# wlsdzyzl/OnePiece

Hardware: AMD Instinct MI355X
Metric: RGB-D frames/sec fused (640x480, 5 mm voxel TSDF) (higher is better)
Workload: dtype f32

## Files before the change

### onepiece_amd/csrc/integrate.hip

```cpp
#include "volume_core.hpp"

namespace {

typedef unsigned int kc_v2u __attribute__((ext_vector_type(2)));

__device__ __forceinline__ void voxel_load(const float* p, float& s, float& w, float& c0, float& c1, float& c2) {
    s = p[0]; w = p[kVox]; c0 = p[2 * kVox]; c1 = p[3 * kVox]; c2 = p[4 * kVox];
}
__device__ __forceinline__ void voxel_store(float* p, float s, float w, float c0, float c1, float c2) {
    p[0] = s; p[kVox] = w; p[2 * kVox] = c0; p[3 * kVox] = c1; p[4 * kVox] = c2;
}
template <bool PLAIN, bool LEAN = false>
__device__ __forceinline__ void voxel_update(float& s, float& w, float& c0, float& c1, float& c2, float new_sdf, unsigned rgba, const float* s_c255) {
    const float n0 = s_c255[rgba & 0xffu], n1 = s_c255[(rgba >> 8) & 0xffu], n2 = s_c255[(rgba >> 16) & 0xffu];
    if (PLAIN) {
        const float wv = LEAN ? w : ((s >= 1 || w <= 0) ? 0.0f : w);
        const float ps = wv * s, p0 = wv * c0, p1 = wv * c1, p2 = wv * c2;
        const float wsum = wv + 1.0f;
        const float y = __builtin_amdgcn_rcpf(wsum);
        const float ns = ps + 1.0f * new_sdf;
        const float m0 = p0 + 1.0f * n0, m1 = p1 + 1.0f * n1, m2 = p2 + 1.0f * n2;
        float qs = div_int_rcp(ns, wsum, y), q0 = div_int_rcp(m0, wsum, y), q1 = div_int_rcp(m1, wsum, y), q2 = div_int_rcp(m2, wsum, y);
        const bool slow = LEAN ? !(fabsf(ns) >= 0x1p-60f) : ((wsum > 0x1p19f) | !(fabsf(ns) >= 0x1p-60f));
        if (__builtin_expect(__builtin_amdgcn_ballot_w64(slow) != 0ull, 0)) {
            if (slow) { qs = ns / wsum; q0 = m0 / wsum; q1 = m1 / wsum; q2 = m2 / wsum; }
        }
        s = qs; c0 = q0; c1 = q1; c2 = q2;
        w = wsum;
    } else if (!(s >= 1 || w <= 0)) {
        const float wsum = w + 1.0f;
        s = (w * s + 1.0f * new_sdf) / wsum;
        c0 = (w * c0 + 1.0f * n0) / wsum;
        c1 = (w * c1 + 1.0f * n1) / wsum;
        c2 = (w * c2 + 1.0f * n2) / wsum;
        w = wsum;
    } else {
        s = new_sdf; w = 1.0f; c0 = n0; c1 = n1; c2 = n2;
    }
}

__device__ __forceinline__ void voxel_revert(bool hit, float& s, float& w, float& c0, float& c1, float& c2, float new_sdf, unsigned rgba, const float* s_c255, bool& can,
                                             bool& zero) {
    can = hit & !(s >= 1 || w <= 0) & (w >= 1);
    const float rw = w + (-1.0f);
    zero = rw == 0;
    if (!can) return;
    const float n0 = s_c255[rgba & 0xffu], n1 = s_c255[(rgba >> 8) & 0xffu], n2 = s_c255[(rgba >> 16) & 0xffu];
    if (zero) {
        s = 999.0f; w = 0.0f; c0 = -1.0f; c1 = -1.0f; c2 = -1.0f;
    } else {
        s = (w * s + (-1.0f) * new_sdf) / rw;
        c0 = (w * c0 + (-1.0f) * n0) / rw;
        c1 = (w * c1 + (-1.0f) * n1) / rw;
        c2 = (w * c2 + (-1.0f) * n2) / rw;
        w = rw;
    }
}

#ifdef KC_TRACE
__device__ unsigned long long g_kc_trace[4096 * 4 * 8];
#define KC_T(K) do { const unsigned long long now_ = __builtin_amdgcn_s_memtime(); kt_[K] += now_ - kt_last_; kt_last_ = now_; } while (0)
#define KC_N(K, V) do { kt_[K] += (V); } while (0)
#else
#define KC_T(K) do { } while (0)
#define KC_N(K, V) do { } while (0)
#endif
template <bool FAST, bool PLAIN, int ZT, bool SUMF = false, bool LEAN = false, bool G2D = false, bool SIGNED = false>
__global__ __launch_bounds__(512 / ZT, (SUMF ? KC_SUM_MIN_WAVES : SIGNED ? KC_SIGNED_MIN_WAVES : KC_COL_MIN_WAVES)) void k_integrate(BatchInv B, CamParams C, VolView V, const uint2* __restrict__ pimg, State* st,
                                                                            int n_frames, unsigned long long* __restrict__ upd_partial,
                                                                            unsigned long long* __restrict__ sel_partial, unsigned long long* __restrict__ chg_partial,
                                                                            unsigned plain_from, unsigned* __restrict__ rc_sum, unsigned rc_stamp, bmask_t sign,
                                                                            unsigned long long* __restrict__ dei_partial) {
    static_assert(!SIGNED || !(PLAIN || SUMF || LEAN), "the PLAIN and LEAN hypotheses do not survive a weight of -1");
    constexpr int kWaves = 8 / ZT;
    constexpr bool kSummaries = !SUMF && !SIGNED;
    constexpr bool kWCount = LEAN && !SUMF;
    __shared__ unsigned s_cnt[kWaves][SIGNED ? 5 : 2];
    __shared__ unsigned s_sign[2][kWaves];
    __shared__ float s_c255[256];
    __shared__ unsigned s_next[2];
    const unsigned long long t_in = __builtin_amdgcn_s_memtime();
#ifdef KC_TRACE
    unsigned long long kt_[8] = {0, 0, 0, 0, 0, 0, 0, 0}, kt_last_ = t_in;
#endif
    for (unsigned k = blockIdx.x * blockDim.x + threadIdx.x; k < (unsigned)(kMaxBatch * kAccSlots * 8); k += gridDim.x * blockDim.x) (&st->acc[0][0][0])[k] = 0u;
    if (st->overflow & 3u) return;
    const int tid = threadIdx.x, lane = tid & 63, zg = tid >> 6;
    if (!SUMF) for (int k = tid; k < 256; k += blockDim.x) s_c255[k] = (float)k / 255.0f;
    const unsigned npix = (unsigned)(C.width * C.height);
    const float half = C.res / 2;
    const float ox = (float)(lane & 7) * C.res + half;
    const float oy = (float)(lane >> 3) * C.res + half;
    const float __attribute__((address_space(4)))* kargs =
        (const float __attribute__((address_space(4)))*)__builtin_amdgcn_kernarg_segment_ptr();
    (void)B;
    unsigned upd = 0, sel = 0, chg = 0, nblk = 0;
    unsigned neg_hit = 0, neg_can = 0, rst = 0;
    const bool eighths = n_frames >= KC_STEAL_MIN_FRAMES;
    constexpr unsigned kChunkLog2 = 5u, kChunk = 1u << kChunkLog2;
    const unsigned n0 = st->n_blist < V.max_blocks ? st->n_blist : V.max_blocks;
    const unsigned n_chunks = (n0 + kChunk - 1u) >> kChunkLog2;
    const unsigned per0 = eighths ? (n0 + (unsigned)kKcShares - 1u) / (unsigned)kKcShares : ((n_chunks + (unsigned)kKcShares - 1u) / (unsigned)kKcShares) << kChunkLog2;
    unsigned xcd = blockIdx.x % (unsigned)kKcShares;
    for (;;) {
    unsigned* ctr = &st->kc_next[xcd * 16u];
    if (tid == 0) s_next[0] = atomicAdd(ctr, 1u);
    __syncthreads();
    unsigned slot = 0u;
    for (unsigned j = s_next[0]; j < per0;) {
        if (tid == 0) s_next[slot ^ 1u] = atomicAdd(ctr, 1u);
        const unsigned b = eighths ? xcd * per0 + j : (((j >> kChunkLog2) * (unsigned)kKcShares + xcd) << kChunkLog2) + (j & (kChunk - 1u));
        KC_T(0);
        const int tslot = b < n0 ? V.blist[b] : -1;
        const int idx = tslot >= 0 ? V.tvals[tslot] : -1;
        KC_N(6, 1);
        if (idx >= 0) {
            const bmask_t mask = V.bmask[tslot];
            if (zg == 0) { sel += mask_popc(mask); ++nblk; }
            const int kx = V.keys[3 * idx], ky = V.keys[3 * idx + 1], kz = V.keys[3 * idx + 2];
            float* vox = V.pool + (size_t)idx * kBlockFloats + (zg * ZT) * 64 + lane;
            float s[ZT], w[ZT], c0[ZT], c1[ZT], c2[ZT], pz[ZT];
#pragma unroll
            for (int z = 0; z < ZT; ++z) {
                if (!SUMF) voxel_load(vox + z * 64, s[z], w[z], c0[z], c1[z], c2[z]);
                pz[z] = ((float)kz * 8.0f) * C.res + ((float)(zg * ZT + z) * C.res + half);
            }
            const float px = ((float)kx * 8.0f) * C.res + ox;
            const float py = ((float)ky * 8.0f) * C.res + oy;
            float w0[ZT];
#pragma unroll
            for (int z = 0; z < ZT; ++z) w0[z] = kWCount ? w[z] : 0.0f;
            unsigned changed = 0u;
            unsigned long long changed_m[ZT];
#pragma unroll
            for (int z = 0; z < ZT; ++z) changed_m[z] = 0ull;
            float ssum[ZT];
            unsigned acc02[ZT], acc1n[ZT];
#pragma unroll
            for (int z = 0; z < ZT; ++z) { ssum[z] = 0.0f; acc02[z] = 0u; acc1n[z] = 0u; }
            auto project = [&](int f, kc_v2u (&rec)[ZT], float (&zc)[ZT]) {
                int fo = f;
                asm volatile("" : "+s"(fo));
                const float __attribute__((address_space(4)))* M = kargs + fo * 12;
                const char* fbase = (const char*)pimg + (unsigned)fo * (npix * 8u);
                const __amdgpu_buffer_rsrc_t frame = __builtin_amdgcn_make_buffer_rsrc((void*)fbase, 0, (int)(npix * 8u), 0x00020000);
                const px_v4i frame2d = gather2d_rsrc(fbase, C.width, C.height);
                const float a0 = M[0] * px + M[1] * py, a1 = M[4] * px + M[5] * py, a2 = M[8] * px + M[9] * py;
#pragma unroll
                for (int z = 0; z < ZT; ++z) {
                    const float q0 = (a0 + M[2] * pz[z]) + M[3] * 1.0f;
                    const float q1 = (a1 + M[6] * pz[z]) + M[7] * 1.0f;
                    const float q2 = (a2 + M[10] * pz[z]) + M[11] * 1.0f;
                    zc[z] = q2;
                    if (G2D) {
                        int u, v;
                        project_pixel_uv<FAST>(C, q0, q1, q2, u, v);
                        rec[z] = gather2d(frame2d, u, v, C.width);
                    } else {
                        const int pix = project_pixel<FAST>(C, q0, q1, q2);
                        rec[z] = __builtin_amdgcn_raw_buffer_load_b64(frame, pix * 8, 0, 0);
                    }
                }
            };
            const bool plain_block = PLAIN || (unsigned)idx >= plain_from;
            auto apply = [&](const kc_v2u (&rec)[ZT], const float (&zc)[ZT], auto plain_c, bool negative) {
                constexpr bool kPlain = decltype(plain_c)::value;
#pragma unroll
                for (int z = 0; z < ZT; ++z) {
                    const float d = __uint_as_float(rec[z].x);
                    const float new_sdf = d - zc[z];
                    const bool seen = d > 0, near = fabsf(new_sdf) < C.trunc, hit = seen & near;
                    if constexpr (SIGNED) {
                        if (negative) {
                            bool can, zero;
                            voxel_revert(hit, s[z], w[z], c0[z], c1[z], c2[z], new_sdf, rec[z].y, s_c255, can, zero);
                            const unsigned long long m_can = __builtin_amdgcn_ballot_w64(can);
                            neg_hit += (unsigned)__builtin_popcountll(__builtin_amdgcn_ballot_w64(seen) & __builtin_amdgcn_ballot_w64(near));
                            neg_can += (unsigned)__builtin_popcountll(m_can);
                            rst += (unsigned)__builtin_popcountll(m_can & __builtin_amdgcn_ballot_w64(zero));
                            changed_m[z] |= m_can;
                            continue;
                        }
                    }
                    if (kWCount) {
                        if (hit) voxel_update<true, true>(s[z], w[z], c0[z], c1[z], c2[z], new_sdf, rec[z].y, s_c255);
                        continue;
                    }
                    const unsigned long long hits = __builtin_amdgcn_ballot_w64(seen) & __builtin_amdgcn_ballot_w64(near);
                    upd += (unsigned)__builtin_popcountll(hits);
                    if (SUMF) {
                        ssum[z] += hit ? new_sdf : 0.0f;
                        const unsigned t = hit ? rec[z].y : 0u;
                        acc02[z] += t & 0x00ff00ffu;
                        acc1n[z] += (t >> 8) & 0x00ff00ffu;
                    } else {
                        changed_m[z] |= hits;
                        if (hit) voxel_update<kPlain, kPlain && LEAN>(s[z], w[z], c0[z], c1[z], c2[z], new_sdf, rec[z].y, s_c255);
                    }
                }
            };
            kc_v2u recA[ZT], recB[ZT];
            float zcA[ZT], zcB[ZT];
            bool negA = false, negB = false;
#ifdef KC_TRACE
            { float keep_ = px + py + pz[0]; if (!SUMF) keep_ += s[0]; asm volatile("" :: "v"(keep_)); KC_T(1); }
#endif
            auto frames = [&](auto plain_c) {
                bmask_t m = mask;
                if (!m) return;
                int f = mask_ctz(m); m &= m - 1u;
                project(f, recA, zcA);
                if constexpr (SIGNED) negA = ((sign >> f) & 1u) != 0u;
                for (;;) {
                    const bool more1 = m != 0u;
                    if (more1) {
                        f = mask_ctz(m); m &= m - 1u; project(f, recB, zcB);
                        if constexpr (SIGNED) negB = ((sign >> f) & 1u) != 0u;
                    }
                    apply(recA, zcA, plain_c, negA);
                    if (!more1) break;
                    const bool more2 = m != 0u;
                    if (more2) {
                        f = mask_ctz(m); m &= m - 1u; project(f, recA, zcA);
                        if constexpr (SIGNED) negA = ((sign >> f) & 1u) != 0u;
                    }
                    apply(recB, zcB, plain_c, negB);
                    if (!more2) break;
                }
            };
            if constexpr (SIGNED) frames(std::false_type{});
            else if (SUMF || PLAIN || plain_block) frames(std::true_type{}); else frames(std::false_type{});
            KC_T(2); KC_N(7, mask_popc(mask));
            if (SUMF) {
#pragma unroll
                for (int z = 0; z < ZT; ++z)
                    if (acc1n[z] >> 16) voxel_load(vox + z * 64, s[z], w[z], c0[z], c1[z], c2[z]);
#pragma unroll
                for (int z = 0; z < ZT; ++z) {
                    const unsigned cnt = acc1n[z] >> 16;
                    if (cnt) {
                        changed |= 1u << z;
                        const bool valid = !(s[z] >= 1 || w[z] <= 0);
                        const float wv = valid ? w[z] : 0.0f, nf = (float)cnt, wsum = wv + nf;
                        const float b0 = (float)(acc02[z] & 0xffffu) / 255.0f, b1 = (float)(acc1n[z] & 0xffffu) / 255.0f, b2 = (float)(acc02[z] >> 16) / 255.0f;
                        s[z] = ((valid ? wv * s[z] : 0.0f) + ssum[z]) / wsum;
                        c0[z] = ((valid ? wv * c0[z] : 0.0f) + b0) / wsum;
                        c1[z] = ((valid ? wv * c1[z] : 0.0f) + b1) / wsum;
                        c2[z] = ((valid ? wv * c2[z] : 0.0f) + b2) / wsum;
                        w[z] = wsum;
                    }
                }
            }
            if (kWCount) {
#pragma unroll
                for (int z = 0; z < ZT; ++z) {
                    const bool wrote = w[z] != w0[z];
                    upd += (unsigned)(w[z] - w0[z]);
                    chg += (unsigned)__builtin_popcountll(__builtin_amdgcn_ballot_w64(wrote));
                    if (wrote) voxel_store(vox + z * 64, s[z], w[z], c0[z], c1[z], c2[z]);
                }
            } else {
#pragma unroll
                for (int z = 0; z < ZT; ++z)
                    if (SUMF ? ((changed >> z) & 1u) != 0u : ((changed_m[z] >> lane) & 1ull) != 0ull) voxel_store(vox + z * 64, s[z], w[z], c0[z], c1[z], c2[z]);
                if (SUMF) chg += (unsigned)__popc(changed);
                else {
#pragma unroll
                    for (int z = 0; z < ZT; ++z) chg += (unsigned)__builtin_popcountll(changed_m[z]);
                }
            }
            if (kSummaries && rc_sum) {
                bool neg = false, pos = false;
#pragma unroll
                for (int z = 0; z < ZT; ++z) { const bool obs = w[z] > 0; neg |= obs && s[z] <= 0; pos |= obs && s[z] > 0; }
                const unsigned f = (__builtin_amdgcn_ballot_w64(neg) ? 1u : 0u) | (__builtin_amdgcn_ballot_w64(pos) ? 2u : 0u);
                if (lane == 0) s_sign[slot][zg] = f;
            }
        }
        KC_T(3);
        __syncthreads();
        KC_T(4);
        if (tslot >= 0 && tid == 0) V.bmask[tslot] = (bmask_t)0;
        if (kSummaries && rc_sum && idx >= 0 && tid == 0) {
            unsigned f = 0u;
#pragma unroll
            for (int k = 0; k < kWaves; ++k) f |= s_sign[slot][k];
            rc_sum[idx] = (rc_stamp << 2) | f;
        }
        slot ^= 1u;
        j = s_next[slot];
    }
    if (!eighths) break;
    __syncthreads();
    if (tid < 64) {
        unsigned left = 0u;
        if (tid < kKcShares) {
            const unsigned c = __hip_atomic_load(&st->kc_next[(unsigned)tid * 16u], __ATOMIC_RELAXED, __HIP_MEMORY_SCOPE_AGENT);
            left = c < per0 ? per0 - c : 0u;
        }
        unsigned key = ((left < 0x7fffffu ? left : 0x7fffffu) << 8) | (unsigned)tid;
#pragma unroll
        for (int o = 32; o > 0; o >>= 1) { const unsigned x = __shfl_xor(key, o, 64); key = x > key ? x : key; }
        if (tid == 0) s_next[0] = key;
    }
    __syncthreads();
    const unsigned key = s_next[0];
    if ((key >> 8) == 0u) break;
    xcd = key & 0xffu;
    __syncthreads();
    }
#ifdef KC_TRACE
    KC_T(5);
    if (lane == 0 && blockIdx.x < 4096) for (int k = 0; k < 8; ++k) g_kc_trace[((size_t)blockIdx.x * 4 + zg) * 8 + k] = kt_[k];
#endif
    if (SUMF) chg = wave_sum(chg);
    if (kWCount) upd = wave_sum(upd);
    if (lane == 0) { s_cnt[zg][0] = upd; s_cnt[zg][1] = chg; }
    if constexpr (SIGNED) if (lane == 0) { s_cnt[zg][2] = neg_can - rst; s_cnt[zg][3] = rst; s_cnt[zg][4] = neg_hit - neg_can; }
    __syncthreads();
    if (tid == 0) {
        unsigned t = 0, c = 0;
        for (int k = 0; k < kWaves; ++k) { t += s_cnt[k][0]; c += s_cnt[k][1]; }
        const unsigned slot_c = blockIdx.x % (unsigned)kPartialGrid;
        if constexpr (SIGNED) {
            unsigned d[3] = {0, 0, 0};
            for (int k = 0; k < kWaves; ++k)
                for (int q = 0; q < 3; ++q) d[q] += s_cnt[k][2 + q];
            atomicAdd(&dei_partial[kDeiReverted + slot_c], (unsigned long long)d[0]);
            atomicAdd(&dei_partial[kDeiReset + slot_c], (unsigned long long)d[1]);
            atomicAdd(&dei_partial[kDeiSkipped + slot_c], (unsigned long long)d[2]);
            if (blockIdx.x == 0) dei_partial[kDeiFrames] += (unsigned long long)mask_popc(sign);
        }
        atomicAdd(&upd_partial[slot_c], (unsigned long long)t);
        atomicAdd(&sel_partial[slot_c], (unsigned long long)sel);
        atomicAdd(&chg_partial[slot_c], (unsigned long long)c);
        atomicAdd(&chg_partial[kPartialGrid + slot_c], (unsigned long long)nblk);
        if (blockIdx.x == 0) { st->stat_frames += (unsigned long long)n_frames; st->stat_launches += 1ull; }
        atomicMax(&st->kc_t[blockIdx.x % (unsigned)kKcTSlots], (unsigned long long)__builtin_amdgcn_s_memtime() - t_in);
    }
}

__global__ __launch_bounds__(256) void k_debug_voxel_update(const float* __restrict__ s, const float* __restrict__ w, const float* __restrict__ c0, const float* __restrict__ c1,
                                                            const float* __restrict__ c2, const float* __restrict__ new_sdf, const unsigned* __restrict__ rgba, long long n,
                                                            float* __restrict__ out_fast, float* __restrict__ out_ref) {
    __shared__ float s_c255[256];
    s_c255[threadIdx.x] = (float)threadIdx.x / 255.0f;
    __syncthreads();
    const long long i = blockIdx.x * 256ll + threadIdx.x;
    if (i >= n) return;
    float a[5] = {s[i], w[i], c0[i], c1[i], c2[i]}, b[5] = {a[0], a[1], a[2], a[3], a[4]};
    voxel_update<true>(a[0], a[1], a[2], a[3], a[4], new_sdf[i], rgba[i], s_c255);
    voxel_update<false>(b[0], b[1], b[2], b[3], b[4], new_sdf[i], rgba[i], s_c255);
    for (int k = 0; k < 5; ++k) { out_fast[5 * i + k] = a[k]; out_ref[5 * i + k] = b[k]; }
}
__global__ void k_debug_rcp(const float* __restrict__ x, long long n, float* __restrict__ out) {
    const long long i = blockIdx.x * 256ll + threadIdx.x;
    if (i < n) out[i] = __builtin_amdgcn_rcpf(x[i]);
}
__global__ void k_debug_gather2d(const uint2* __restrict__ img, int width, int height, int frame, int column_test, const int* __restrict__ uv, long long n,
                                 uint2* __restrict__ out) {
    const long long i = blockIdx.x * 256ll + threadIdx.x;
    if (i >= n) return;
    int fo = frame;
    asm volatile("" : "+s"(fo));
    const px_v4i rsrc = gather2d_rsrc(img + (size_t)fo * ((size_t)width * height), width, height);
    const px_v2u r = column_test ? gather2d(rsrc, uv[2 * i], uv[2 * i + 1], width) : op_struct_buffer_load_b64(rsrc, uv[2 * i + 1], uv[2 * i] << 3, 0, 0);
    out[i] = make_uint2(r.x, r.y);
}

}

namespace opv {

bool vol_fusion_keeps_summaries(const op_volume* v) {
    const bool sum_form = v->update_mode == OP_VOLUME_UPDATE_SUM_FORM && v->trunc < 1.0f;
    return !sum_form && v->rc_sum != nullptr && v->rc_cap >= v->max_blocks && (v->content_gen >> 30) == v->rc_sum_epoch;
}

enum { kUpdSum, kUpdLean, kUpdPlain, kUpdGeneral, kUpdSigned };
enum { kGatExact, kGatFastRaw, kGatFast2d };
template <int UPD, int GAT>
void launch_kc(op_volume* v, const BatchInv& I, const CamParams& C, int nf, bmask_t sign, unsigned* rc_sum) {
    constexpr bool kSum = UPD == kUpdSum, kSigned = UPD == kUpdSigned;
    constexpr int kZt = kSum ? KC_ZT_SUM : KC_ZT;
    hipLaunchKernelGGL((k_integrate<GAT != kGatExact, (UPD <= kUpdPlain), kZt, kSum, UPD == kUpdLean, GAT == kGatFast2d, kSigned>),
                       dim3(kSum ? kColGridSum : kSigned ? kSignedGrid : kColGrid), dim3(512 / kZt), 0, v->stream, I, C, v->view(), (const uint2*)v->pimg, v->state, nf,
                       v->upd_partial, v->sel_partial, v->chg_partial, v->plain_from, rc_sum, (unsigned)(v->content_gen & 0x3fffffffull), sign, v->dei_partial);
}

void launch_integrate(op_volume* v, const BatchInv& I, const CamParams& C, int nf, bmask_t sign) {
    const bool sum_form = !sign && v->update_mode == OP_VOLUME_UPDATE_SUM_FORM && v->trunc < 1.0f;
    unsigned* rc_sum = !sign && vol_fusion_keeps_summaries(v) ? v->rc_sum : nullptr;
    if (sum_form || !(v->trunc <= 0.5f)) v->lean_ok = false;
    v->lean_frames += (uint64_t)nf;
    const bool lean = v->plain && v->lean_ok && v->lean_frames <= (1ull << 19);
    const int upd = sign ? kUpdSigned : sum_form ? kUpdSum : lean ? kUpdLean : v->plain ? kUpdPlain : kUpdGeneral;
    const int gat = !C.fast_px ? kGatExact : gather2d_fits(C.width) ? kGatFast2d : kGatFastRaw;
    typedef void (*launch_fn)(op_volume*, const BatchInv&, const CamParams&, int, bmask_t, unsigned*);
    static const launch_fn table[5][3] = {
        {launch_kc<kUpdSum, kGatExact>, launch_kc<kUpdSum, kGatFastRaw>, launch_kc<kUpdSum, kGatFast2d>},
        {launch_kc<kUpdLean, kGatExact>, launch_kc<kUpdLean, kGatFastRaw>, launch_kc<kUpdLean, kGatFast2d>},
        {launch_kc<kUpdPlain, kGatExact>, launch_kc<kUpdPlain, kGatFastRaw>, launch_kc<kUpdPlain, kGatFast2d>},
        {launch_kc<kUpdGeneral, kGatExact>, launch_kc<kUpdGeneral, kGatFastRaw>, launch_kc<kUpdGeneral, kGatFast2d>},
        {launch_kc<kUpdSigned, kGatExact>, launch_kc<kUpdSigned, kGatFastRaw>, launch_kc<kUpdSigned, kGatFast2d>}};
    table[upd][gat](v, I, C, nf, sign, rc_sum);
}

void kc_trace_dump(op_volume* v) {
#ifdef KC_TRACE
    if (hipSetDevice(v->device) == hipSuccess && hipDeviceSynchronize() == hipSuccess) {
        const int nw = kColGrid * (8 / KC_ZT);
        std::vector<unsigned long long> t((size_t)4096 * 4 * 8);
        if (hipMemcpyFromSymbol(t.data(), HIP_SYMBOL(g_kc_trace), t.size() * 8) == hipSuccess) {
            double sum[8] = {0}, mx[8] = {0};
            for (int w = 0; w < nw; ++w)
                for (int k = 0; k < 8; ++k) { const double d = (double)t[(size_t)w * 8 + k]; sum[k] += d; mx[k] = std::max(mx[k], d); }
            const double n = nw;
            fprintf(stderr, "kc trace (shader cycles per wave of the last launch, %d waves; mean/max): draw+list %.0f/%.0f metadata+voxels %.0f/%.0f frames %.0f/%.0f stores %.0f/%.0f barrier %.0f/%.0f tail %.0f/%.0f | blocks %.1f/%.0f frames applied %.0f/%.0f\n",
                    nw, sum[0] / n, mx[0], sum[1] / n, mx[1], sum[2] / n, mx[2], sum[3] / n, mx[3], sum[4] / n, mx[4], sum[5] / n, mx[5], sum[6] / n, mx[6], sum[7] / n, mx[7]);
        }
    }
#else
    (void)v;
#endif
#ifdef OP_PX_TRACE
    unsigned long long pw[2] = {0, 0};
    if (hipSetDevice(v->device) == hipSuccess && hipDeviceSynchronize() == hipSuccess && hipMemcpyFromSymbol(pw, HIP_SYMBOL(g_px_waves), sizeof(pw)) == hipSuccess)
        fprintf(stderr, "px trace (k_integrate, since load): %llu wave-projections, %llu took the exact fallback (%.3f %%)\n", pw[0], pw[1],
                pw[0] ? 100.0 * (double)pw[1] / (double)pw[0] : 0.0);
#endif
}

}

extern "C" {

int op_debug_voxel_update(const float* s, const float* w, const float* c0, const float* c1, const float* c2, const float* new_sdf, const unsigned* rgba, long long n,
                          float* out_fast, float* out_ref) {
    if (!s || !w || !c0 || !c1 || !c2 || !new_sdf || !rgba || !out_fast || !out_ref) return fail(OP_ERR_INVALID, "null argument");
    if (n < 0 || n > (1ll << 28)) return fail(OP_ERR_INVALID, "n out of range [0, 2^28]");
    OP_TRY(op::use_device(0));
    if (n == 0) return OP_OK;
    const size_t N = (size_t)n;
    float* d_in = nullptr;
    float* d_out = nullptr;
    OP_HIP(op::cached_malloc((void**)&d_in, 7 * N * 4));
    hipError_t e = op::cached_malloc((void**)&d_out, 10 * N * 4);
    const void* src[7] = {s, w, c0, c1, c2, new_sdf, rgba};
    for (int k = 0; k < 7 && e == hipSuccess; ++k) e = hipMemcpy(d_in + k * N, src[k], N * 4, hipMemcpyHostToDevice);
    if (e == hipSuccess) {
        hipLaunchKernelGGL(k_debug_voxel_update, dim3((unsigned)((N + 255) / 256)), dim3(256), 0, 0, (const float*)d_in, (const float*)(d_in + N), (const float*)(d_in + 2 * N),
                           (const float*)(d_in + 3 * N), (const float*)(d_in + 4 * N), (const float*)(d_in + 5 * N), (const unsigned*)(d_in + 6 * N), n, d_out, d_out + 5 * N);
        e = hipMemcpy(out_fast, d_out, 5 * N * 4, hipMemcpyDeviceToHost);
        if (e == hipSuccess) e = hipMemcpy(out_ref, d_out + 5 * N, 5 * N * 4, hipMemcpyDeviceToHost);
    }
    op::cached_free(d_in);
    if (d_out) op::cached_free(d_out);
    if (e != hipSuccess) return fail(OP_ERR_HIP, "op_debug_voxel_update failed: %s", hipGetErrorString(e));
    return OP_OK;
}

int op_debug_rcp(const float* x, long long n, float* out) {
    if (!x || !out) return fail(OP_ERR_INVALID, "null argument");
    if (n < 0 || n > (1ll << 28)) return fail(OP_ERR_INVALID, "n out of range [0, 2^28]");
    OP_TRY(op::use_device(0));
    if (n == 0) return OP_OK;
    const size_t N = (size_t)n;
    float* d = nullptr;
    OP_HIP(op::cached_malloc((void**)&d, 2 * N * 4));
    hipError_t e = hipMemcpy(d, x, N * 4, hipMemcpyHostToDevice);
    if (e == hipSuccess) {
        hipLaunchKernelGGL(k_debug_rcp, dim3((unsigned)((N + 255) / 256)), dim3(256), 0, 0, (const float*)d, n, d + N);
        e = hipMemcpy(out, d + N, N * 4, hipMemcpyDeviceToHost);
    }
    op::cached_free(d);
    if (e != hipSuccess) return fail(OP_ERR_HIP, "op_debug_rcp failed: %s", hipGetErrorString(e));
    return OP_OK;
}

double op_debug_px_rcp_err(void) { return kPxRcpErr; }

int op_debug_gather2d(const unsigned* images, int width, int height, int n_frames, int frame, int column_test, const int* uv, long long n, unsigned* out) {
    if (!images || !uv || !out) return fail(OP_ERR_INVALID, "null argument");
    if (width <= 0 || !gather2d_fits(width) || height <= 0 || n_frames <= 0 || frame < 0 || frame >= n_frames || (long long)width * height * n_frames > (1ll << 24))
        return fail(OP_ERR_INVALID, "op_debug_gather2d: rows of 1 .. %d pixels, a frame of the stack, at most 2^24 pixels in all", kGather2dMaxWidth);
    if (n < 0 || n > (1ll << 24)) return fail(OP_ERR_INVALID, "n out of range [0, 2^24]");
    for (long long i = 0; i < 2 * n; ++i)
        if (uv[i] < -(1 << 23) || uv[i] >= (1 << 23)) return fail(OP_ERR_INVALID, "op_debug_gather2d: coordinates in [-2^23, 2^23)");
    if (!column_test)
        for (long long i = 0; i < n; ++i) {
            const long long rec = ((long long)frame * height + uv[2 * i + 1]) * width + uv[2 * i];
            if (rec < 0 || rec >= (long long)width * height * n_frames) return fail(OP_ERR_INVALID, "op_debug_gather2d: without the column test every address must lie in the stack");
        }
    OP_TRY(op::use_device(0));
    if (n == 0) return OP_OK;
    const size_t N = (size_t)n, img_bytes = (size_t)width * height * n_frames * 8;
    char* d = nullptr;
    OP_HIP(op::cached_malloc((void**)&d, img_bytes + 16 * N));
    hipError_t e = hipMemcpy(d, images, img_bytes, hipMemcpyHostToDevice);
    if (e == hipSuccess) e = hipMemcpy(d + img_bytes, uv, 8 * N, hipMemcpyHostToDevice);
    if (e == hipSuccess) {
        hipLaunchKernelGGL(k_debug_gather2d, dim3((unsigned)((N + 255) / 256)), dim3(256), 0, 0, (const uint2*)d, width, height, frame, column_test, (const int*)(d + img_bytes), n,
                           (uint2*)(d + img_bytes + 8 * N));
        e = hipMemcpy(out, d + img_bytes + 8 * N, 8 * N, hipMemcpyDeviceToHost);
    }
    op::cached_free(d);
    if (e != hipSuccess) return fail(OP_ERR_HIP, "op_debug_gather2d failed: %s", hipGetErrorString(e));
    return OP_OK;
}

}
```

Before: 58200.

## Map each wave onto an 8x4x2 voxel sub-box instead of one z-slice

```diff
diff --git a/onepiece_amd/csrc/integrate.hip b/onepiece_amd/csrc/integrate.hip
--- a/onepiece_amd/csrc/integrate.hip
+++ b/onepiece_amd/csrc/integrate.hip
@@ -1,4 +1,5 @@
 #include "volume_core.hpp"
+#include "kc_lanes.hpp"
 
 namespace {
 
@@ -89,8 +90,9 @@
     if (!SUMF) for (int k = tid; k < 256; k += blockDim.x) s_c255[k] = (float)k / 255.0f;
     const unsigned npix = (unsigned)(C.width * C.height);
     const float half = C.res / 2;
-    const float ox = (float)(lane & 7) * C.res + half;
-    const float oy = (float)(lane >> 3) * C.res + half;
+    const int lx = kc_lanes::vx<ZT>(zg, 0, lane), ly = kc_lanes::vy<ZT>(zg, 0, lane), lz = kc_lanes::vz<ZT>(zg, 0, lane);
+    const float ox = (float)lx * C.res + half;
+    const float oy = (float)ly * C.res + half;
     const float __attribute__((address_space(4)))* kargs =
         (const float __attribute__((address_space(4)))*)__builtin_amdgcn_kernarg_segment_ptr();
     (void)B;
@@ -118,12 +120,12 @@
             const bmask_t mask = V.bmask[tslot];
             if (zg == 0) { sel += mask_popc(mask); ++nblk; }
             const int kx = V.keys[3 * idx], ky = V.keys[3 * idx + 1], kz = V.keys[3 * idx + 2];
-            float* vox = V.pool + (size_t)idx * kBlockFloats + (zg * ZT) * 64 + lane;
+            float* vox = V.pool + (size_t)idx * kBlockFloats + (lx + 8 * ly + 64 * lz);
             float s[ZT], w[ZT], c0[ZT], c1[ZT], c2[ZT], pz[ZT];
 #pragma unroll
             for (int z = 0; z < ZT; ++z) {
-                if (!SUMF) voxel_load(vox + z * 64, s[z], w[z], c0[z], c1[z], c2[z]);
-                pz[z] = ((float)kz * 8.0f) * C.res + ((float)(zg * ZT + z) * C.res + half);
+                if (!SUMF) voxel_load(vox + z * kc_lanes::kSlotStride, s[z], w[z], c0[z], c1[z], c2[z]);
+                pz[z] = ((float)kz * 8.0f) * C.res + ((float)(lz + z * kc_lanes::kBZ) * C.res + half);
             }
             const float px = ((float)kx * 8.0f) * C.res + ox;
             const float py = ((float)ky * 8.0f) * C.res + oy;
@@ -234,7 +236,7 @@
             if (SUMF) {
 #pragma unroll
                 for (int z = 0; z < ZT; ++z)
-                    if (acc1n[z] >> 16) voxel_load(vox + z * 64, s[z], w[z], c0[z], c1[z], c2[z]);
+                    if (acc1n[z] >> 16) voxel_load(vox + z * kc_lanes::kSlotStride, s[z], w[z], c0[z], c1[z], c2[z]);
 #pragma unroll
                 for (int z = 0; z < ZT; ++z) {
                     const unsigned cnt = acc1n[z] >> 16;
@@ -257,12 +259,12 @@
                     const bool wrote = w[z] != w0[z];
                     upd += (unsigned)(w[z] - w0[z]);
                     chg += (unsigned)__builtin_popcountll(__builtin_amdgcn_ballot_w64(wrote));
-                    if (wrote) voxel_store(vox + z * 64, s[z], w[z], c0[z], c1[z], c2[z]);
+                    if (wrote) voxel_store(vox + z * kc_lanes::kSlotStride, s[z], w[z], c0[z], c1[z], c2[z]);
                 }
             } else {
 #pragma unroll
                 for (int z = 0; z < ZT; ++z)
-                    if (SUMF ? ((changed >> z) & 1u) != 0u : ((changed_m[z] >> lane) & 1ull) != 0ull) voxel_store(vox + z * 64, s[z], w[z], c0[z], c1[z], c2[z]);
+                    if (SUMF ? ((changed >> z) & 1u) != 0u : ((changed_m[z] >> lane) & 1ull) != 0ull) voxel_store(vox + z * kc_lanes::kSlotStride, s[z], w[z], c0[z], c1[z], c2[z]);
                 if (SUMF) chg += (unsigned)__popc(changed);
                 else {
 #pragma unroll
diff --git a/onepiece_amd/csrc/kc_lanes.hpp b/onepiece_amd/csrc/kc_lanes.hpp
--- /dev/null
+++ b/onepiece_amd/csrc/kc_lanes.hpp
@@ -0,0 +1,17 @@
+#pragma once
+
+namespace kc_lanes {
+
+constexpr int kBX = 8, kBY = 4, kBZ = 2;
+constexpr int kNY = 8 / kBY, kNZ = 8 / kBZ;
+static_assert(kBX * kBY * kBZ == 64 && 8 % kBX == 0 && 8 % kBY == 0 && 8 % kBZ == 0, "a wave's lanes fill one sub-box of the block");
+constexpr int kSlotStride = 64 * kBZ;
+constexpr int kRun = kBX == 8 ? 8 * kBY : kBX;
+
+template <int ZT> constexpr int box(int wave, int slot) { static_assert(kNZ % ZT == 0, "a thread's slots are sub-boxes behind one another"); return wave * ZT + slot; }
+template <int ZT> constexpr int vx(int wave, int slot, int lane) { return box<ZT>(wave, slot) / (kNZ * kNY) * kBX + lane % kBX; }
+template <int ZT> constexpr int vy(int wave, int slot, int lane) { return box<ZT>(wave, slot) / kNZ % kNY * kBY + lane / kBX % kBY; }
+template <int ZT> constexpr int vz(int wave, int slot, int lane) { return box<ZT>(wave, slot) % kNZ * kBZ + lane / (kBX * kBY); }
+template <int ZT> constexpr int offset(int wave, int slot, int lane) { return vx<ZT>(wave, slot, lane) + 8 * vy<ZT>(wave, slot, lane) + 64 * vz<ZT>(wave, slot, lane); }
+
+}
```

Result: faster. 59080 (median of 6 runs) (+1.5%).
